# excamera/alfalfa

Measured on NVIDIA H100. Metric: decode_throughput, higher is better.
Workload: dtype u8

## Files before the change

### alfalfa_b200/csrc/encoder.cu

```cuda
#include <cuda_runtime.h>
#include <stdio.h>
#include <stdlib.h>
#include <string.h>

#include <algorithm>
#include <chrono>
#include <condition_variable>
#include <mutex>
#include <string>
#include <utility>
#include <vector>

#include "../../include/vp8gpu.h"
#include "enc_costs.h"
#include "engine.hpp"
#include "hostpool.h"
#include "parser.h"
#include "serializer.h"
#include "vp8_enc_tables.h"
#include "vp8_tables.h"

using vp8::Engine;

extern "C" Engine* vp8gpu_ctx_engine(vp8gpu_ctx* ctx);
// ... 262 lines not shown
  if (late) {
    ft.late_loop_filter_level = &LateLevel::wait;
    ft.late_ctx = late;
  }
  bytes = vp8::serialize_frame(h, enc->h_mbs, enc->h_tokens, nullptr, &ft);
  if (bytes.empty()) return e->fail(VP8GPU_ERR_LOGIC, "serializer rejected the device records");
  return VP8GPU_OK;
}

int filter_frame(vp8gpu_encoder* enc, int frame, bool key, int level) {
  Engine* e = enc->e;
  const vp8::Geom& g = e->geom();
  cudaStream_t s = e->stream(enc->lane);
  if (level <= 0) return VP8GPU_OK;
  vp8::DevJob* dj = reinterpret_cast<vp8::DevJob*>(enc->h_hdr + 512);
  memset(dj, 0, 512);
  int* d_sync = reinterpret_cast<int*>(enc->dev + enc->off_sync);
  dj->mbs = reinterpret_cast<const vp8gpu_mb*>(enc->dev + enc->off_mbs);
  dj->tokens = reinterpret_cast<const vp8gpu_token*>(enc->dev + enc->off_tokens);
  dj->out = e->frame_dev(frame);
  dj->lf_progress = d_sync + 128 + g.mb_rows;
  dj->intra_progress = d_sync + 128;
  dj->key_frame = key;
  dj->sharpness = (uint8_t)enc->lf_sharpness;
  dj->lf_enabled = 1;
  dj->lf_force = (uint8_t)level;
  int ids[1] = {frame};
  int rc = e->acquire_frames(enc->lane, ids, 1);
  if (rc != VP8GPU_OK) return rc;
  CUE(cudaMemcpyAsync(enc->dev + enc->off_encjob + 512, dj, 512, cudaMemcpyHostToDevice, s));
  CUE(cudaMemsetAsync(d_sync + 32, 0, sizeof(int), s));
  CUE(cudaMemsetAsync(d_sync + 128 + g.mb_rows, 0, sizeof(int) * (size_t)g.mb_rows, s));
  const vp8::DevJob* d_dj = reinterpret_cast<const vp8::DevJob*>(enc->dev + enc->off_encjob + 512);
  if (int ce = vp8::launch_loopfilter(d_dj, 1, g, d_sync + 32, e->next_epoch(2), s)) return e->cuda_fail((cudaError_t)ce, "k_loopfilter");
  e->count_launches(1);
  e->mark_frames(enc->lane, ids, 1);
  CUE(cudaStreamSynchronize(s));
  return VP8GPU_OK;
}

int filter_batch(vp8gpu_encoder* enc, const int* frames, const int* levels, int n, bool key) {
  Engine* e = enc->e;
  const vp8::Geom& g = e->geom();
  cudaStream_t s = e->stream(enc->lane);
  if (n <= 0) return VP8GPU_OK;
  if (n > kLfMax) return e->fail(VP8GPU_ERR_LOGIC, "filter_batch: too many trials");
  vp8::DevJob* dj = reinterpret_cast<vp8::DevJob*>(enc->h_hdr + 512);
  memset(dj, 0, sizeof(vp8::DevJob) * n);
  int* d_sync = reinterpret_cast<int*>(enc->dev + enc->off_sync);
  for (int i = 0; i < n; i++) {
    dj[i].mbs = reinterpret_cast<const vp8gpu_mb*>(enc->dev + enc->off_mbs);
    dj[i].tokens = reinterpret_cast<const vp8gpu_token*>(enc->dev + enc->off_tokens);
    dj[i].out = e->frame_dev(frames[i]);
    dj[i].lf_progress = d_sync + 128 + (size_t)(1 + i) * g.mb_rows;
    dj[i].intra_progress = d_sync + 128;
    dj[i].key_frame = key;
    dj[i].sharpness = (uint8_t)enc->lf_sharpness;
    dj[i].lf_enabled = 1;
    dj[i].lf_force = (uint8_t)levels[i];
  }
  int rc = e->acquire_frames(enc->lane, frames, n);
  if (rc != VP8GPU_OK) return rc;
  CUE(cudaMemcpyAsync(enc->dev + enc->off_encjob + 512, dj, sizeof(vp8::DevJob) * n, cudaMemcpyHostToDevice, s));
  CUE(cudaMemsetAsync(d_sync + 32, 0, sizeof(int), s));
  CUE(cudaMemsetAsync(d_sync + 128 + g.mb_rows, 0, sizeof(int) * (size_t)n * g.mb_rows, s));
  const vp8::DevJob* d_dj = reinterpret_cast<const vp8::DevJob*>(enc->dev + enc->off_encjob + 512);
  if (int ce = vp8::launch_loopfilter(d_dj, n, g, d_sync + 32, e->next_epoch(2), s)) return e->cuda_fail((cudaError_t)ce, "k_loopfilter");
  e->count_launches(1);
  e->mark_frames(enc->lane, frames, n);
  CUE(cudaStreamSynchronize(s));
  return VP8GPU_OK;
}

bool enc_speculate() {
  static const bool on = [] {
    const char* v = getenv("VP8GPU_ENC_SPECULATE");
    return !(v && v[0] == '0');
  }();
  return on;
}

int choose_loop_filter(vp8gpu_encoder* enc, int* recon, bool key, int* level_out, double* ssim_out) {
  Engine* e = enc->e;
  int lo = 0, hi = 63;
  if (enc->last_lf >= 0) {
    lo = enc->last_lf > 0 ? enc->last_lf - 1 : 0;
    hi = enc->last_lf + 1 > 63 ? 63 : enc->last_lf + 1;
  }
  int temps[kLfMax], n_temps = 0;
  const int want = enc_speculate() ? (hi - lo + 1 < kLfMax ? hi - lo + 1 : kLfMax) : 1;
  for (; n_temps < want; n_temps++)
    if (e->frame_alloc(&temps[n_temps]) != VP8GPU_OK) break;
  if (n_temps == 0) return e->fail(VP8GPU_ERR_NOMEM, "loop-filter search: no raster for a trial");
  int best = 0, keep = -1;
  double best_ssim = -1.0;
  int rc = VP8GPU_OK;
  bool stop = false, found = false;
  for (int level = lo; level <= hi && !stop && rc == VP8GPU_OK;) {
    int use[kLfMax], lv[kLfMax], n = 0, nf = 0, fr[kLfMax], fl[kLfMax];
    for (int i = 0; i < n_temps && level + n <= hi; i++) {
// ... 1294 lines not shown
```

### alfalfa_b200/csrc/engine.cu

```cuda
#include "engine.hpp"

#include <cuda.h>
#include <stdlib.h>
#include <string.h>

namespace vp8 {

int launch_compare(const uint8_t* a, const uint8_t* b, const Geom& g, int* d_flag, void* stream);
int launch_hash(const uint8_t* a, const Geom& g, unsigned long long* d_out, void* stream);

namespace {
inline size_t align_up(size_t v, size_t a) { return (v + a - 1) / a * a; }

std::mutex g_tmap_mu;
struct TmapChunk {
  uint8_t* base;
  size_t used, cap;
};
std::vector<TmapChunk> g_tmap_chunks[64];
uint8_t* tmap_arena_alloc(int device, size_t bytes) {
  std::lock_guard<std::mutex> lk(g_tmap_mu);
  if (device < 0 || device >= 64) return nullptr;
  auto& chunks = g_tmap_chunks[device];
  if (chunks.empty() || chunks.back().used + bytes > chunks.back().cap) {
// ... 465 lines not shown
    if (jobs[i].ring) {
      L.mbs_off.push_back(0);
      L.tok_off.push_back(0);
      L.split_off.push_back(0);
      continue;
    }
    L.mbs_off.push_back(off);
    off = align_up(off + n_mbs * sizeof(vp8gpu_mb), 256);
    L.tok_off.push_back(off);
    off = align_up(off + (size_t)jobs[i].desc->n_tokens * sizeof(vp8gpu_token) + 4, 256);
    L.split_off.push_back(off);
    off = align_up(off + (size_t)jobs[i].desc->n_split * sizeof(vp8gpu_split_mvs) + 4, 256);
  }
  L.total = off;
  return L;
}
}

int Engine::build_and_launch(int lane, const DevJob* d_jobs, int* d_sync, int n, bool any_inter, bool any_intra,
                             bool any_lf, cudaEvent_t* between) {
  cudaStream_t s = lanes_[lane];
  if (between) CU(cudaEventRecord(between[2], s));
  if (any_inter) {
    if (int e = launch_inter(d_jobs, n, g_, s)) return cuda_fail((cudaError_t)e, "k_inter launch");
    launches_++;
  }
  if (between) CU(cudaEventRecord(between[0], s));
  if (any_intra) {
    if (int e = launch_intra(d_jobs, n, g_, d_sync + 0, next_epoch(1), s)) return cuda_fail((cudaError_t)e, "k_intra launch");
    launches_++;
  }
  if (between) CU(cudaEventRecord(between[1], s));
  if (any_lf) {
    if (int e = launch_loopfilter(d_jobs, n, g_, d_sync + 32, next_epoch(2), s)) return cuda_fail((cudaError_t)e, "k_loopfilter launch");
    launches_++;
  }
  return VP8GPU_OK;
}

uint32_t Engine::token_cap_for(size_t bits) const {
  const size_t by_bytes = align_up(bits + 16, 256) * 9 + 1024, by_blocks = (size_t)g_.mb_cols * g_.mb_rows * 400;
  return (uint32_t)(by_bytes < by_blocks ? by_bytes : by_blocks);
}

TokenRing Engine::token_ring_layout(size_t max_frame_bytes, bool arena) const {
  const size_t n_mbs = (size_t)g_.mb_cols * g_.mb_rows;
  TokenRing r;
  r.bits_cap = (uint32_t)align_up(max_frame_bytes + 16, 256);
  r.split_cap = (uint32_t)n_mbs;
  r.tok_cap = token_cap_for(max_frame_bytes);
  size_t off = 256;
  r.probs_off = off;
  off += 1280;
  r.info_off = off;
  off = align_up(off + 4 * ((n_mbs + 15) / 16 + 1), 256);
  r.bits_off = off;
  off = align_up(off + r.bits_cap, 256);
  r.host_stride = off;
  r.result_off = off;
  off += 256;
  r.above_off = off;
  off = align_up(off + 2 * (size_t)g_.mb_cols, 256);
  r.mbs_off = off;
  off = align_up(off + n_mbs * sizeof(vp8gpu_mb), 256);
  r.split_off = off;
  off = align_up(off + (size_t)r.split_cap * sizeof(vp8gpu_split_mvs), 256);
  r.tok_off = off;
// ... 414 lines not shown
```

### alfalfa_b200/csrc/engine.h

```cpp
#pragma once
#include <stdint.h>

#include "../../include/vp8gpu.h"

#ifdef VP8GPU_SIMT_EMUL
#define VP8_LAUNCH(kern, grid, block, smem, stream) ::simt::make_launch((grid), (block), (smem), [](auto... a_) { kern(a_...); })
#else
#define VP8_LAUNCH(kern, grid, block, smem, stream) kern<<<(grid), (block), (smem), (stream)>>>
#endif

namespace vp8 {

struct Geom {
  int mb_cols, mb_rows;
  int W, H;
  int y_pitch, c_pitch;
  uint32_t u_off, v_off;
  uint32_t frame_bytes;
  uint32_t msg_lf_off, msg_intra_off;
  uint32_t alloc_bytes;
};

struct DevJob {
  const vp8gpu_mb* mbs;
// ... 39 lines not shown
};

struct ReencJob {
  const uint8_t* target;
  uint8_t* recon;
  const vp8gpu_mb* mbs_in;
  vp8gpu_mb* mbs_out;
  vp8gpu_token* tokens;
  uint32_t* tok_counter;
  uint32_t tok_cap;
  int* progress;
  vp8gpu_quant q;
  uint16_t cols, rows;
};

struct TokJob {
  vp8gpu_mb* mbs;
  vp8gpu_token* tokens;
  const uint8_t* bits;
  const uint8_t* coef_probs;
  uint32_t* result;
  uint16_t* above;
  const uint32_t* mbinfo;
  uint32_t part_off[8], part_len[8];
  uint32_t nparts;
  uint32_t tok_cap;
};

int launch_inter(const DevJob* jobs, int njobs, const Geom& g, void* stream);
int launch_enc_rd_trellis(const EncJob* job, int rows, const Geom& g, int* ticket, void* stream);
int launch_reenc_inter(const ReencJob* jobs, int njobs, int n_mbs, const Geom& g, void* stream);
int launch_reenc_intra(const ReencJob* jobs, int njobs, int rows, const Geom& g, int* ticket, void* stream);
int launch_intra(const DevJob* jobs, int njobs, const Geom& g, int* ticket, uint32_t epoch, void* stream);
int launch_loopfilter(const DevJob* jobs, int njobs, const Geom& g, int* ticket, uint32_t epoch, void* stream);
int launch_tokens(const uint8_t* ring, size_t stride, int first, int count, int nslots, const Geom& g, void* stream);
int launch_fetch_header(void* dst, const void* src_host_devptr, size_t bytes, void* stream);
int launch_ssim(const uint8_t* a, const uint8_t* b, const Geom& g, float* d_windows, void* stream);
int launch_enc_rd(const EncJob* jobs, int njobs, int rows, const Geom& g, int* ticket, void* stream);

}
```

### alfalfa_b200/csrc/engine.hpp

```cpp
#pragma once
#include <cuda_runtime.h>
#include <stdint.h>

#include <atomic>
#include <mutex>
#include <string>
#include <vector>

#include "engine.h"
#include "parser.h"

namespace vp8 {

constexpr int kMaxLanes = 32;
constexpr int kStagingDepth = 3;

struct TokenRing {
  int nslots = 0;
  uint8_t* dev = nullptr;
  uint8_t* host = nullptr;
  size_t stride = 0, host_stride = 0;
  size_t probs_off = 0, info_off = 0, bits_off = 0, result_off = 0, above_off = 0, mbs_off = 0, split_off = 0, tok_off = 0;
  uint32_t bits_cap = 0, split_cap = 0, tok_cap = 0;
  vp8gpu_token* arena = nullptr;
// ... 15 lines not shown
  cudaEvent_t consumed = nullptr;
  const TokenRing* ring = nullptr;
  int ring_slot = 0;
  cudaEvent_t ready = nullptr;
  cudaEvent_t* finished = nullptr;
};

class Engine {
 public:
  static int create(int device, int width, int height, int max_frames, Engine** out, std::string* err);
  ~Engine();

  const Geom& geom() const { return g_; }
  int width() const { return width_; }
  int height() const { return height_; }
  int device() const { return device_; }

  int frame_alloc(int* id);
  int frame_retain(int id);
  int frame_release(int id);
  int frames_free();
  int frames_in_use() {
    std::lock_guard<std::mutex> lk(mu_);
    int n = 0;
    for (const Frame& f : frames_) n += f.refcnt > 0;
    return n;
  }
  uint32_t next_epoch(int kernel_bit = 3) {
    if (!(ll_mask_ & kernel_bit)) return 0;
    uint32_t e = ++epoch_;
    if (e == 0) e = ++epoch_;
    return e;
  }
  int frame_upload(int id, const uint8_t* y, size_t ys, const uint8_t* u, const uint8_t* v, size_t cs);
  int frame_download(int id, uint8_t* y, size_t ys, uint8_t* u, uint8_t* v, size_t cs);
  int frame_download_display(int id, int lane, uint8_t* dst, size_t dst_size, bool wait);
  int frames_download_display(const int* ids, uint8_t* const* dsts, int n, int lane);
  int frame_clear(int id, int lane);
  int frame_copy(int dst, int src, int lane);
  int frame_copy_raw(int id, void* buf, size_t bytes, bool into_frame);
  int frames_equal(int a, int b, int lane, int* equal);
  int frame_hash(int id, int lane, uint64_t* out);
  int frames_ssim(int a, int b, int lane, double* out);

  int submit(int lane, const HostJob* jobs, int n, cudaEvent_t consumed, cudaEvent_t* between = nullptr);

  TokenRing token_ring_layout(size_t max_frame_bytes, bool arena = false) const;
  uint32_t token_cap_for(size_t bits) const;
  int token_ring_create(int nslots, size_t max_frame_bytes, TokenRing** out, size_t arena_tokens = 0);
  void token_ring_free(TokenRing* r);
  int token_ring_stage(TokenRing* r, int slot, const ParsedFrame& f, cudaStream_t s, vp8gpu_token* tokens = nullptr);
  int token_ring_launch(TokenRing* r, int first, int count, cudaStream_t s);
  int token_ring_clear_result(TokenRing* r, int slot, cudaStream_t s);
  int token_ring_result(TokenRing* r, int slot, cudaStream_t s, uint32_t result[2]);

  struct Resident;
  int resident_upload(const HostJob* jobs, int n, Resident** out);
  int resident_run(int lane, Resident* r, float* ms);
  int resident_run_many(int lane, Resident* const* rs, int n, float* total_ms);
  int resident_run_timed(int lane, Resident* r, float ms[3]);
  void resident_free(Resident* r);

  uint8_t* frame_dev(int id) { return frames_[id].dev; }
  const void* frame_tmaps(int id) const { return tmaps_ ? tmaps_ + (size_t)id * 384 : nullptr; }
  int acquire_frames(int lane, const int* ids, int n, uint32_t write_mask = ~0u);
  int mark_frames(int lane, const int* ids, int n, uint32_t write_mask = ~0u);
// ... 26 lines not shown
    uint8_t* host_dev = nullptr;
    size_t host_cap = 0;
    cudaEvent_t done = nullptr;
    bool in_flight = false;
  };
  static constexpr int kEventRing = 2048;
  cudaEvent_t next_event(int slot);
  int touch(Frame& f, int slot, bool write = true, cudaEvent_t shared = nullptr);
  void collect_waits(const Frame& f, int slot, bool write, std::vector<cudaEvent_t>& out) const;
  int wait_for(Frame& f, int slot, cudaStream_t s, bool write = true);
  int build_and_launch(int lane, const DevJob* d_jobs, int* d_sync, int n, bool any_inter, bool any_intra,
                       bool any_lf, cudaEvent_t* between = nullptr);
  int count_jobs(const HostJob& j, uint32_t* n_intra, uint32_t* n_inter, uint32_t* n_filtered) const;

  int device_ = 0, width_ = 0, height_ = 0;
  Geom g_{};
  std::mutex mu_;
  std::vector<Frame> frames_;
  std::vector<int> free_;
  cudaStream_t lanes_[2 * kMaxLanes] = {};
  cudaEvent_t ring_[2 * kMaxLanes][kEventRing] = {};
  int ring_next_[2 * kMaxLanes] = {};
  Staging staging_[kMaxLanes][kStagingDepth];
  int staging_next_[kMaxLanes] = {};
  uint8_t* cmp_scratch_ = nullptr;
  float* ssim_dev_[kMaxLanes] = {};
  float* ssim_host_[kMaxLanes] = {};
  uint8_t* tmaps_ = nullptr;
  int make_tensor_maps(int id);
  std::atomic<uint64_t> launches_{0};
  std::string err_;
  std::mutex err_mu_;
  std::atomic<uint32_t> epoch_{0};
  int ll_mask_ = 1;
};

}
```

### alfalfa_b200/csrc/kernels.cu

```cuda
#include <cuda_runtime.h>
#include <stdint.h>

#include "enc_costs.h"
#include "engine.h"
#include "vp8_math.cuh"

namespace vp8 {
namespace {

#define VP8_LUT_QUALIFIER __device__ const
#include "bpred_lut.inc"

__constant__ int16_t c_sixtap[8][6] = {{0, 0, 128, 0, 0, 0},     {0, -6, 123, 12, -1, 0}, {2, -11, 108, 36, -8, 1},
                                      {0, -9, 93, 50, -6, 0},   {3, -16, 77, 77, -16, 3}, {0, -6, 50, 93, -9, 0},
                                      {1, -8, 36, 108, -11, 2}, {0, -1, 12, 123, -6, 0}};

#ifdef VP8_PROFILE
__device__ unsigned long long g_prof[32];
#define PROF_DECL unsigned long long prof_t = clock64(), prof_acc[8] = {0, 0, 0, 0, 0, 0, 0, 0}; unsigned prof_n = 0
#define PROF(i)                                  \
  do {                                           \
    const unsigned long long now_ = clock64();   \
    prof_acc[i] += now_ - prof_t;                \
    prof_t = now_;                               \
// ... 564 lines not shown
        else d = pix + 256 + 64 * ((b - 16) >> 2) + (((b >> 1) & 1) * 4) * 8 + (b & 1) * 4 + 2 * cp, ds = 8;
        const uint8_t* m = &S.s.mid[b][0][2 * cp];
        if (fy) {
          vitem<4>(m, 4, c_sixtap[fy], d, ds);
        } else {
#pragma unroll
          for (int j = 0; j < 4; j++) *reinterpret_cast<uint16_t*>(d + j * ds) = *reinterpret_cast<const uint16_t*>(m + (j + 2) * 4);
        }
      }
    }
    __syncwarp();
  }

  if (nz) add_residuals(pix, S.coef, nz, S.nzlist, lane);
  store_mb(pix, J.out, g, col, row, lane);
}

#ifndef VP8GPU_SIMT_EMUL
__device__ __forceinline__ int ld_progress(const int* p) {
  int v;
  asm volatile("ld.acquire.gpu.global.s32 %0, [%1];" : "=r"(v) : "l"(p) : "memory");
  return v;
}
__device__ __forceinline__ void st_progress(int* p, int v) {
  asm volatile("st.release.gpu.global.s32 [%0], %1;" ::"l"(p), "r"(v) : "memory");
}
#else
__device__ __forceinline__ int ld_progress(const int* p) {
  simt::yield();
  return *reinterpret_cast<const volatile int*>(p);
}
__device__ __forceinline__ void st_progress(int* p, int v) { *reinterpret_cast<volatile int*>(p) = v; }
#endif
__device__ __forceinline__ void wait_row(const int* progress_above, int need, int lane) {
  if (lane == 0) {
    unsigned ns = 20;
    while (ld_progress(progress_above) < need) {
      __nanosleep(ns);
      if (ns < 160) ns += ns;
    }
  }
  __syncwarp();
}
__device__ __forceinline__ void publish_row(int* progress, int value, int lane) {
  __syncwarp();
  if (lane == 0) st_progress(progress, value);
}
__device__ __forceinline__ uint8_t ldcg_u8(const uint8_t* p) { return __ldcg(p); }

__device__ __forceinline__ int next_marked(uint32_t my_word, int from, int nwords) {
  for (int w = from >> 5; w < nwords; w++) {
    uint32_t bits = __shfl_sync(0xffffffffu, my_word, w);
    if (w == (from >> 5)) bits &= 0xffffffffu << (from & 31);
    if (bits) return w * 32 + __ffs(bits) - 1;
  }
  return -1;
}

constexpr int WS = 48;

__device__ __forceinline__ void add_residuals_intra(uint8_t* W, uint8_t* pixc, const int16_t* coef, int lane,
                                                    bool luma_too) {
  for (int g4 = (luma_too ? lane : 64 + lane); g4 < 96; g4 += 32) {
    int blk, ry;
    uint8_t* p;
    if (g4 < 64) {
// ... 217 lines not shown
      *reinterpret_cast<uint2*>((plane ? V : U) + (size_t)(8 * row + yy) * g.c_pitch + 8 * col) =
          *reinterpret_cast<const uint2*>(pixc + plane * 64 + yy * 8);
    }
    const int next = next_marked(my_word, col + 1, nwords);
    PROF(5);
    publish_row(progress, next < 0 ? cols : next, lane);
    PROF(6);
    PROF_COUNT();
    col = next;
  }
  PROF_FLUSH(0);
}

__device__ __forceinline__ void filter_edge_at(int* px, int q, const vp8m::LfParams& lp, bool mb_edge) {
  const int mask = vp8m::lf_mask(lp.interior, mb_edge ? lp.mb_edge : lp.sub_edge, px[q - 4], px[q - 3], px[q - 2],
                                 px[q - 1], px[q], px[q + 1], px[q + 2], px[q + 3]);
  if (!mask) return;
  const int hev = vp8m::lf_hev(lp.hev, px[q - 2], px[q - 1], px[q], px[q + 1]);
  if (mb_edge) vp8m::lf_mbedge(mask, hev, px[q - 3], px[q - 2], px[q - 1], px[q], px[q + 1], px[q + 2]);
  else vp8m::lf_inner(mask, hev, px[q - 2], px[q - 1], px[q], px[q + 1]);
}
__device__ __forceinline__ void filter_line(int* px, bool luma, bool do_mb_edge, bool do_inner,
                                            const vp8m::LfParams& lp) {
  if (do_mb_edge) filter_edge_at(px, 4, lp, true);
  if (do_inner) {
    filter_edge_at(px, 8, lp, false);
    if (luma) {
      filter_edge_at(px, 12, lp, false);
      filter_edge_at(px, 16, lp, false);
    }
  }
}

__global__ void __launch_bounds__(32 * WF_WARPS, 16) k_loopfilter(const DevJob* __restrict__ jobs, int njobs, Geom g, int* ticket) {
  constexpr int YS = 20, CSZ = 12;
  __shared__ __align__(16) uint8_t s_ry[WF_WARPS][20 * YS];
  __shared__ __align__(16) uint8_t s_rc[WF_WARPS][2][12 * CSZ];
  const int lane = threadIdx.x & 31, warp = threadIdx.x >> 5;
  uint8_t* const ry = s_ry[warp];
  uint8_t (*const rc)[12 * CSZ] = s_rc[warp];
  int t = 0;
  if (lane == 0) t = atomicAdd(ticket, 1);
  t = __shfl_sync(0xffffffffu, t, 0);
  const int row = t / njobs, job = t - row * njobs;
  if (row >= g.mb_rows) return;
  const DevJob& J = jobs[job];
  if (!J.lf_enabled) return;
  const int cols = g.mb_cols;
  const vp8gpu_mb* row_mbs = J.mbs + (size_t)row * cols;

  const int nwords = (cols + 31) >> 5;
  uint32_t my_word = 0;
  for (int w = 0; w < nwords; w++) {
    const int c = w * 32 + lane;
    const bool filtered = c < cols && (J.lf_force || ((__ldg(reinterpret_cast<const uint32_t*>(row_mbs + c) + 2) >> 16) & 0xFF) != 0);
    const uint32_t bits = __ballot_sync(0xffffffffu, filtered);
    if (lane == w) my_word = bits;
  }
  int col = next_marked(my_word, 0, nwords);
  int* progress = J.lf_progress + row;
  publish_row(progress, col < 0 ? cols : col, lane);

  uint8_t* const Y = J.out;
  uint8_t* const U = J.out + g.u_off;
  uint8_t* const V = J.out + g.v_off;
  const int y_lo = row > 0 ? 0 : 4;
// ... 48 lines not shown
        if (lane < 20) left0 = *reinterpret_cast<const uint32_t*>(ry + lane * YS + 16);
        if (lane < 24) left1 = *reinterpret_cast<const uint32_t*>(rc[lane / 12] + (lane % 12) * CSZ + 8);
      } else {
        if (lane < 20 && lane >= y_lo)
          left0 = __ldcg(reinterpret_cast<const uint32_t*>(Y + (size_t)(16 * row - 4 + lane) * g.y_pitch + 16 * col - 4));
        if (lane < 24 && (lane % 12) >= y_lo)
          left1 = __ldcg(reinterpret_cast<const uint32_t*>((lane / 12 ? V : U) + (size_t)(8 * row - 4 + lane % 12) * g.c_pitch + 8 * col - 4));
      }
    }
    __syncwarp();
    if (col > 0) {
      if (lane < 20) *reinterpret_cast<uint32_t*>(ry + lane * YS) = left0;
      if (lane < 24) *reinterpret_cast<uint32_t*>(rc[lane / 12] + (lane % 12) * CSZ) = left1;
    }
    if (row > 0) {
      if (lane < 16) *reinterpret_cast<uint32_t*>(ry + (lane >> 2) * YS + 4 + 4 * (lane & 3)) = top;
      else {
        const int cw = lane - 16, plane = cw >> 3, k2 = cw & 7;
        *reinterpret_cast<uint32_t*>(rc[plane] + (k2 >> 1) * CSZ + 4 + 4 * (k2 & 1)) = top;
      }
    }
#pragma unroll
    for (int k = 0; k < 3; k++) {
      const uint8_t* gp;
      uint8_t* sp;
      own_ptr(k, col, gp, sp);
      *reinterpret_cast<uint32_t*>(sp) = own[k];
    }
    __syncwarp();
    PROF(2);
    const int next = next_marked(my_word, col + 1, nwords);
    if (next >= 0) prefetch_own(next);

    const vp8m::LfParams lp = vp8m::lf_params(J.lf_force ? J.lf_force : f.lf_level, J.sharpness, J.key_frame);
    const bool do_inner = !((f.flags & VP8GPU_MB_HAS_Y2) && f.tok_cnt == 0);
    const bool luma = lane < 16;
    uint8_t* const plane_base = luma ? ry : rc[(lane - 16) >> 3];
    const int stride = luma ? YS : CSZ, idx = luma ? lane : (lane & 7), len = luma ? 20 : 12;
    int px[20];

    {
      const uint32_t* rw = reinterpret_cast<const uint32_t*>(plane_base + (4 + idx) * stride);
#pragma unroll
      for (int k = 0; k < 5; k++) {
        const uint32_t v = (k < 3 || luma) ? rw[k] : 0u;
        px[4 * k] = v & 0xFF, px[4 * k + 1] = (v >> 8) & 0xFF, px[4 * k + 2] = (v >> 16) & 0xFF, px[4 * k + 3] = v >> 24;
      }
      filter_line(px, luma, col > 0, do_inner, lp);
      uint32_t* ww = reinterpret_cast<uint32_t*>(plane_base + (4 + idx) * stride);
#pragma unroll
      for (int k = 0; k < 5; k++)
        if (k < 3 || luma) ww[k] = (uint32_t)px[4 * k] | ((uint32_t)px[4 * k + 1] << 8) | ((uint32_t)px[4 * k + 2] << 16) | ((uint32_t)px[4 * k + 3] << 24);
    }
    __syncwarp();
    {
      uint8_t* cp = plane_base + 4 + idx;
#pragma unroll
      for (int k = 0; k < 20; k++) px[k] = k < len ? cp[k * stride] : 0;
      filter_line(px, luma, row > 0, do_inner, lp);
#pragma unroll
      for (int k = 1; k < 19; k++)
        if (k < len - 1) cp[k * stride] = (uint8_t)px[k];
    }
    __syncwarp();

    PROF(3);
    const int x_lo = col > 0 ? 0 : 1;
    const bool flush_right = next != col + 1;
    {
      uint8_t* const gy = Y + (size_t)(16 * row - 4) * g.y_pitch + 16 * col - 4;
#pragma unroll
      for (int k = 0; k < 3; k++) {
        const int w = lane + 32 * k, r = w >> 2, wx = w & 3;
        if (w < 80 && r >= y_lo && wx >= x_lo)
          *reinterpret_cast<uint32_t*>(gy + (size_t)r * g.y_pitch + 4 * wx) = *reinterpret_cast<const uint32_t*>(ry + r * YS + 4 * wx);
      }
#pragma unroll
      for (int k = 0; k < 2; k++) {
        const int w = lane + 32 * k, plane = w >= 24, kk = w - 24 * plane, r = kk >> 1, wx = kk & 1;
        if (w < 48 && r >= y_lo && wx >= x_lo)
          *reinterpret_cast<uint32_t*>((plane ? V : U) + (size_t)(8 * row - 4 + r) * g.c_pitch + 8 * col - 4 + 4 * wx) =
              *reinterpret_cast<const uint32_t*>(rc[plane] + r * CSZ + 4 * wx);
      }
      if (flush_right) {
        if (lane < 20 && lane >= y_lo)
          *reinterpret_cast<uint32_t*>(gy + (size_t)lane * g.y_pitch + 16) = *reinterpret_cast<const uint32_t*>(ry + lane * YS + 16);
        if (lane < 24) {
          const int plane = lane >= 12, r = lane - 12 * plane;
          if (r >= y_lo)
            *reinterpret_cast<uint32_t*>((plane ? V : U) + (size_t)(8 * row - 4 + r) * g.c_pitch + 8 * col + 4) =
                *reinterpret_cast<const uint32_t*>(rc[plane] + r * CSZ + 8);
        }
      }
    }
    PROF(4);
    publish_row(progress, next < 0 ? cols : next, lane);
    PROF(5);
    PROF_COUNT();
    prev = col;
    col = next;
  }
  PROF_FLUSH(16);
}

#include "wavefront_ll.cuh"

__device__ __forceinline__ int warp_sum(int v) { return __reduce_add_sync(0xffffffffu, v); }
__device__ __forceinline__ uint32_t rdcost(uint32_t rate, uint32_t distortion, uint32_t rm, uint32_t dm) {
  return ((128u + rate * rm) / 256u) + distortion * dm;
}
__device__ __forceinline__ uint32_t variance256(int sum, int sse) {
  const long long s = warp_sum(sum);
  const uint32_t q = (uint32_t)warp_sum(sse);
  return q - (uint32_t)((s * s) / 256);
}

struct __align__(16) EncSmem {
  uint8_t W[17 * WS];
  uint8_t Wb[17 * WS];
  uint8_t src[384];
  uint8_t pcand[2][256];
  uint8_t pixc[128];
  uint8_t tile[21 * 24];
  uint8_t mid[21 * 16];
  int16_t coef[COEF_I16];
  int16_t qb[16][16];
  int16_t tmp[16];
  uint8_t aboveC[2][12];
  uint8_t leftC[2][8];
};
// ... 895 lines not shown
}
__global__ void k_hash(const uint8_t* __restrict__ a, Geom g, unsigned long long* out) {
  const int words_y = g.W / 4, words_c = g.W / 8;
  const int rows_total = g.H + g.H;
  unsigned long long acc = 0;
  for (int r = blockIdx.x; r < rows_total; r += gridDim.x) {
    size_t off;
    int nw;
    if (r < g.H) off = (size_t)r * g.y_pitch, nw = words_y;
    else if (r < g.H + g.H / 2) off = g.u_off + (size_t)(r - g.H) * g.c_pitch, nw = words_c;
    else off = g.v_off + (size_t)(r - g.H - g.H / 2) * g.c_pitch, nw = words_c;
    const uint32_t* pa = reinterpret_cast<const uint32_t*>(a + off);
    for (int i = threadIdx.x; i < nw; i += blockDim.x)
      acc += mix64(((unsigned long long)pa[i] << 32) ^ ((unsigned long long)r << 16) ^ (unsigned long long)i);
  }
  for (int o = 16; o; o >>= 1) acc += __shfl_down_sync(0xffffffffu, acc, o);
  if ((threadIdx.x & 31) == 0 && acc) atomicAdd(out, acc);
}

}

int launch_inter(const DevJob* jobs, int njobs, const Geom& g, void* stream) {
  const int n_mbs = g.mb_cols * g.mb_rows;
  dim3 grid((n_mbs + INTER_WARPS - 1) / INTER_WARPS, njobs);
  VP8_LAUNCH(k_inter, grid, INTER_WARPS * 32, 0, static_cast<cudaStream_t>(stream))(jobs, g);
  return (int)cudaGetLastError();
}
int launch_intra(const DevJob* jobs, int njobs, const Geom& g, int* ticket, uint32_t epoch, void* stream) {
  const int grid = (g.mb_rows * njobs + WF_WARPS - 1) / WF_WARPS;
  if (epoch) VP8_LAUNCH(k_intra_ll, grid, 32 * WF_WARPS, 0, static_cast<cudaStream_t>(stream))(jobs, njobs, g, ticket, epoch);
  else VP8_LAUNCH(k_intra, grid, 32 * WF_WARPS, 0, static_cast<cudaStream_t>(stream))(jobs, njobs, g, ticket);
  return (int)cudaGetLastError();
}
int launch_loopfilter(const DevJob* jobs, int njobs, const Geom& g, int* ticket, uint32_t epoch, void* stream) {
  const int grid = (g.mb_rows * njobs + WF_WARPS - 1) / WF_WARPS;
  if (epoch) VP8_LAUNCH(k_loopfilter_ll, grid, 32 * WF_WARPS, 0, static_cast<cudaStream_t>(stream))(jobs, njobs, g, ticket, epoch);
  else VP8_LAUNCH(k_loopfilter, grid, 32 * WF_WARPS, 0, static_cast<cudaStream_t>(stream))(jobs, njobs, g, ticket);
  return (int)cudaGetLastError();
}

int launch_enc_rd(const EncJob* jobs, int njobs, int rows, const Geom& g, int* ticket, void* stream) {
  VP8_LAUNCH(k_enc_rd<false>, (njobs * rows + WF_WARPS - 1) / WF_WARPS, 32 * WF_WARPS, 0, static_cast<cudaStream_t>(stream))(jobs, njobs, g, ticket);
  return (int)cudaGetLastError();
}
int launch_enc_rd_trellis(const EncJob* job, int rows, const Geom& g, int* ticket, void* stream) {
  VP8_LAUNCH(k_enc_rd<true>, (rows + WF_WARPS - 1) / WF_WARPS, 32 * WF_WARPS, 0, static_cast<cudaStream_t>(stream))(job, 1, g, ticket);
  return (int)cudaGetLastError();
}

int launch_reenc_inter(const ReencJob* jobs, int njobs, int n_mbs, const Geom& g, void* stream) {
  const dim3 grid((n_mbs + REENC_WARPS - 1) / REENC_WARPS, njobs);
  VP8_LAUNCH(k_reenc_inter, grid, 32 * REENC_WARPS, 0, static_cast<cudaStream_t>(stream))(jobs, njobs, g);
  return (int)cudaGetLastError();
}
int launch_reenc_intra(const ReencJob* jobs, int njobs, int rows, const Geom& g, int* ticket, void* stream) {
  VP8_LAUNCH(k_reenc_intra, (njobs * rows + WF_WARPS - 1) / WF_WARPS, 32 * WF_WARPS, 0, static_cast<cudaStream_t>(stream))(jobs, njobs, g, ticket);
  return (int)cudaGetLastError();
}

#ifdef VP8_PROFILE
extern "C" void vp8gpu_debug_profile(unsigned long long out[32], int reset) {
  cudaDeviceSynchronize();
  cudaMemcpyFromSymbol(out, g_prof, sizeof(unsigned long long) * 32);
  if (reset) {
    unsigned long long z[32] = {0};
    cudaMemcpyToSymbol(g_prof, z, sizeof(z));
  }
}
#endif
// ... 31 lines not shown
```

Baseline: 10810.

## Add banded loop-filter kernel passing row edges through shared-memory rings

Adds k_loopfilter_band, in which each CTA filters a band of four consecutive macroblock rows, one warp per row. Filtered bottom edges go to the next warp through a shared-memory ring, and progress is signalled with CTA-scope acquire/release flags instead of global progress counters. Only the band's first and last rows still sync through global memory. The filter body is factored into filter_region so both kernels share it, and the new path is switched on by setting bit 4 of ll_mask_ when the low-latency epoch path is off. The intent is to cut global-memory polling and round trips between adjacent rows, at the cost of extra handshake logic, ring back-pressure stalls and less parallelism per CTA.

```diff
diff --git a/alfalfa_b200/csrc/encoder.cu b/alfalfa_b200/csrc/encoder.cu
--- a/alfalfa_b200/csrc/encoder.cu
+++ b/alfalfa_b200/csrc/encoder.cu
@@ -318,7 +318,7 @@
   CUE(cudaMemsetAsync(d_sync + 32, 0, sizeof(int), s));
   CUE(cudaMemsetAsync(d_sync + 128 + g.mb_rows, 0, sizeof(int) * (size_t)g.mb_rows, s));
   const vp8::DevJob* d_dj = reinterpret_cast<const vp8::DevJob*>(enc->dev + enc->off_encjob + 512);
-  if (int ce = vp8::launch_loopfilter(d_dj, 1, g, d_sync + 32, e->next_epoch(2), s)) return e->cuda_fail((cudaError_t)ce, "k_loopfilter");
+  if (int ce = vp8::launch_loopfilter(d_dj, 1, g, d_sync + 32, e->next_epoch(2), e->lf_band(), s)) return e->cuda_fail((cudaError_t)ce, "k_loopfilter");
   e->count_launches(1);
   e->mark_frames(enc->lane, ids, 1);
   CUE(cudaStreamSynchronize(s));
@@ -351,7 +351,7 @@
   CUE(cudaMemsetAsync(d_sync + 32, 0, sizeof(int), s));
   CUE(cudaMemsetAsync(d_sync + 128 + g.mb_rows, 0, sizeof(int) * (size_t)n * g.mb_rows, s));
   const vp8::DevJob* d_dj = reinterpret_cast<const vp8::DevJob*>(enc->dev + enc->off_encjob + 512);
-  if (int ce = vp8::launch_loopfilter(d_dj, n, g, d_sync + 32, e->next_epoch(2), s)) return e->cuda_fail((cudaError_t)ce, "k_loopfilter");
+  if (int ce = vp8::launch_loopfilter(d_dj, n, g, d_sync + 32, e->next_epoch(2), e->lf_band(), s)) return e->cuda_fail((cudaError_t)ce, "k_loopfilter");
   e->count_launches(1);
   e->mark_frames(enc->lane, frames, n);
   CUE(cudaStreamSynchronize(s));
diff --git a/alfalfa_b200/csrc/engine.cu b/alfalfa_b200/csrc/engine.cu
--- a/alfalfa_b200/csrc/engine.cu
+++ b/alfalfa_b200/csrc/engine.cu
@@ -521,7 +521,7 @@
   }
   if (between) CU(cudaEventRecord(between[1], s));
   if (any_lf) {
-    if (int e = launch_loopfilter(d_jobs, n, g_, d_sync + 32, next_epoch(2), s)) return cuda_fail((cudaError_t)e, "k_loopfilter launch");
+    if (int e = launch_loopfilter(d_jobs, n, g_, d_sync + 32, next_epoch(2), lf_band(), s)) return cuda_fail((cudaError_t)e, "k_loopfilter launch");
     launches_++;
   }
   return VP8GPU_OK;
diff --git a/alfalfa_b200/csrc/engine.h b/alfalfa_b200/csrc/engine.h
--- a/alfalfa_b200/csrc/engine.h
+++ b/alfalfa_b200/csrc/engine.h
@@ -95,7 +95,7 @@
 int launch_reenc_inter(const ReencJob* jobs, int njobs, int n_mbs, const Geom& g, void* stream);
 int launch_reenc_intra(const ReencJob* jobs, int njobs, int rows, const Geom& g, int* ticket, void* stream);
 int launch_intra(const DevJob* jobs, int njobs, const Geom& g, int* ticket, uint32_t epoch, void* stream);
-int launch_loopfilter(const DevJob* jobs, int njobs, const Geom& g, int* ticket, uint32_t epoch, void* stream);
+int launch_loopfilter(const DevJob* jobs, int njobs, const Geom& g, int* ticket, uint32_t epoch, bool band, void* stream);
 int launch_tokens(const uint8_t* ring, size_t stride, int first, int count, int nslots, const Geom& g, void* stream);
 int launch_fetch_header(void* dst, const void* src_host_devptr, size_t bytes, void* stream);
 int launch_ssim(const uint8_t* a, const uint8_t* b, const Geom& g, float* d_windows, void* stream);
diff --git a/alfalfa_b200/csrc/engine.hpp b/alfalfa_b200/csrc/engine.hpp
--- a/alfalfa_b200/csrc/engine.hpp
+++ b/alfalfa_b200/csrc/engine.hpp
@@ -71,6 +71,7 @@
     if (e == 0) e = ++epoch_;
     return e;
   }
+  bool lf_band() const { return ll_mask_ & 4; }
   int frame_upload(int id, const uint8_t* y, size_t ys, const uint8_t* u, const uint8_t* v, size_t cs);
   int frame_download(int id, uint8_t* y, size_t ys, uint8_t* u, uint8_t* v, size_t cs);
   int frame_download_display(int id, int lane, uint8_t* dst, size_t dst_size, bool wait);
@@ -163,7 +164,7 @@
   std::string err_;
   std::mutex err_mu_;
   std::atomic<uint32_t> epoch_{0};
-  int ll_mask_ = 1;
+  int ll_mask_ = 1 | 4;
 };
 
 }
diff --git a/alfalfa_b200/csrc/kernels.cu b/alfalfa_b200/csrc/kernels.cu
--- a/alfalfa_b200/csrc/kernels.cu
+++ b/alfalfa_b200/csrc/kernels.cu
@@ -620,6 +620,36 @@
 }
 __device__ __forceinline__ void st_progress(int* p, int v) { *reinterpret_cast<volatile int*>(p) = v; }
 #endif
+#ifndef VP8GPU_SIMT_EMUL
+__device__ __forceinline__ int ld_flag_cta(const int* p) {
+  int v;
+  asm volatile("ld.acquire.cta.shared::cta.s32 %0, [%1];" : "=r"(v) : "r"((unsigned)__cvta_generic_to_shared(p)) : "memory");
+  return v;
+}
+__device__ __forceinline__ void st_flag_cta(int* p, int v) {
+  asm volatile("st.release.cta.shared::cta.s32 [%0], %1;" ::"r"((unsigned)__cvta_generic_to_shared(p)), "r"(v) : "memory");
+}
+#else
+__device__ __forceinline__ int ld_flag_cta(const int* p) {
+  simt::yield();
+  return *reinterpret_cast<const volatile int*>(p);
+}
+__device__ __forceinline__ void st_flag_cta(int* p, int v) { *reinterpret_cast<volatile int*>(p) = v; }
+#endif
+#ifndef VP8GPU_SIMT_EMUL
+__device__ __forceinline__ int lane_here() {
+  int l;
+  asm volatile("mov.u32 %0, %%laneid;" : "=r"(l));
+  return l;
+}
+#else
+__device__ __forceinline__ int lane_here() { return threadIdx.x & 31; }
+#endif
+__device__ __forceinline__ void wait_flag_cta(const int* flag, int need, int lane) {
+  if (lane == 0)
+    while (ld_flag_cta(flag) < need) __nanosleep(20);
+  __syncwarp();
+}
 __device__ __forceinline__ void wait_row(const int* progress_above, int need, int lane) {
   if (lane == 0) {
     unsigned ns = 20;
@@ -903,6 +933,42 @@
   }
 }
 
+__device__ __forceinline__ void filter_region(uint8_t* ry, uint8_t (*rc)[12 * 12], const DevJob& J, const MbFields& f,
+                                              bool left_edge, bool top_edge, int lane) {
+  constexpr int YS = 20, CSZ = 12;
+  const vp8m::LfParams lp = vp8m::lf_params(J.lf_force ? J.lf_force : f.lf_level, J.sharpness, J.key_frame);
+  const bool do_inner = !((f.flags & VP8GPU_MB_HAS_Y2) && f.tok_cnt == 0);
+  const bool luma = lane < 16;
+  uint8_t* const plane_base = luma ? ry : rc[(lane - 16) >> 3];
+  const int stride = luma ? YS : CSZ, idx = luma ? lane : (lane & 7), len = luma ? 20 : 12;
+  int px[20];
+
+  {
+    const uint32_t* rw = reinterpret_cast<const uint32_t*>(plane_base + (4 + idx) * stride);
+#pragma unroll
+    for (int k = 0; k < 5; k++) {
+      const uint32_t v = (k < 3 || luma) ? rw[k] : 0u;
+      px[4 * k] = v & 0xFF, px[4 * k + 1] = (v >> 8) & 0xFF, px[4 * k + 2] = (v >> 16) & 0xFF, px[4 * k + 3] = v >> 24;
+    }
+    filter_line(px, luma, left_edge, do_inner, lp);
+    uint32_t* ww = reinterpret_cast<uint32_t*>(plane_base + (4 + idx) * stride);
+#pragma unroll
+    for (int k = 0; k < 5; k++)
+      if (k < 3 || luma) ww[k] = (uint32_t)px[4 * k] | ((uint32_t)px[4 * k + 1] << 8) | ((uint32_t)px[4 * k + 2] << 16) | ((uint32_t)px[4 * k + 3] << 24);
+  }
+  __syncwarp();
+  {
+    uint8_t* cp = plane_base + 4 + idx;
+#pragma unroll
+    for (int k = 0; k < 20; k++) px[k] = k < len ? cp[k * stride] : 0;
+    filter_line(px, luma, top_edge, do_inner, lp);
+#pragma unroll
+    for (int k = 1; k < 19; k++)
+      if (k < len - 1) cp[k * stride] = (uint8_t)px[k];
+  }
+  __syncwarp();
+}
+
 __global__ void __launch_bounds__(32 * WF_WARPS, 16) k_loopfilter(const DevJob* __restrict__ jobs, int njobs, Geom g, int* ticket) {
   constexpr int YS = 20, CSZ = 12;
   __shared__ __align__(16) uint8_t s_ry[WF_WARPS][20 * YS];
@@ -1017,37 +1083,7 @@
     const int next = next_marked(my_word, col + 1, nwords);
     if (next >= 0) prefetch_own(next);
 
-    const vp8m::LfParams lp = vp8m::lf_params(J.lf_force ? J.lf_force : f.lf_level, J.sharpness, J.key_frame);
-    const bool do_inner = !((f.flags & VP8GPU_MB_HAS_Y2) && f.tok_cnt == 0);
-    const bool luma = lane < 16;
-    uint8_t* const plane_base = luma ? ry : rc[(lane - 16) >> 3];
-    const int stride = luma ? YS : CSZ, idx = luma ? lane : (lane & 7), len = luma ? 20 : 12;
-    int px[20];
-
-    {
-      const uint32_t* rw = reinterpret_cast<const uint32_t*>(plane_base + (4 + idx) * stride);
-#pragma unroll
-      for (int k = 0; k < 5; k++) {
-        const uint32_t v = (k < 3 || luma) ? rw[k] : 0u;
-        px[4 * k] = v & 0xFF, px[4 * k + 1] = (v >> 8) & 0xFF, px[4 * k + 2] = (v >> 16) & 0xFF, px[4 * k + 3] = v >> 24;
-      }
-      filter_line(px, luma, col > 0, do_inner, lp);
-      uint32_t* ww = reinterpret_cast<uint32_t*>(plane_base + (4 + idx) * stride);
-#pragma unroll
-      for (int k = 0; k < 5; k++)
-        if (k < 3 || luma) ww[k] = (uint32_t)px[4 * k] | ((uint32_t)px[4 * k + 1] << 8) | ((uint32_t)px[4 * k + 2] << 16) | ((uint32_t)px[4 * k + 3] << 24);
-    }
-    __syncwarp();
-    {
-      uint8_t* cp = plane_base + 4 + idx;
-#pragma unroll
-      for (int k = 0; k < 20; k++) px[k] = k < len ? cp[k * stride] : 0;
-      filter_line(px, luma, row > 0, do_inner, lp);
-#pragma unroll
-      for (int k = 1; k < 19; k++)
-        if (k < len - 1) cp[k * stride] = (uint8_t)px[k];
-    }
-    __syncwarp();
+    filter_region(ry, rc, J, f, col > 0, row > 0, lane);
 
     PROF(3);
     const int x_lo = col > 0 ? 0 : 1;
@@ -1081,6 +1117,226 @@
     PROF(4);
     publish_row(progress, next < 0 ? cols : next, lane);
     PROF(5);
+    PROF_COUNT();
+    prev = col;
+    col = next;
+  }
+  PROF_FLUSH(16);
+}
+
+constexpr int LF_BAND = 4, LF_RING = 8;
+
+__global__ void __launch_bounds__(32 * LF_BAND, 32 / LF_BAND) k_loopfilter_band(const DevJob* __restrict__ jobs, int njobs, Geom g, int* ticket) {
+  constexpr int YS = 20, CSZ = 12;
+  struct Row {
+    uint8_t ry[20 * YS];
+    uint8_t rc[2][12 * CSZ];
+    uint32_t ring[LF_RING][32];
+    int done;
+    int free;
+    int pad[2];
+  };
+  __shared__ __align__(16) Row s_rows[LF_BAND];
+  __shared__ int s_ticket;
+  const int lane = threadIdx.x & 31, warp = threadIdx.x >> 5;
+  if (threadIdx.x == 0) s_ticket = atomicAdd(ticket, 1);
+  if (threadIdx.x < LF_BAND) s_rows[threadIdx.x].done = 0, s_rows[threadIdx.x].free = 0;
+  __syncthreads();
+  const int band = s_ticket / njobs, job = s_ticket - band * njobs;
+  const int row = band * LF_BAND + warp;
+  if (row >= g.mb_rows) return;
+  const DevJob& J = jobs[job];
+  if (!J.lf_enabled) return;
+  const int cols = g.mb_cols;
+  const vp8gpu_mb* row_mbs = J.mbs + (size_t)row * cols;
+  Row* const S = s_rows + warp;
+  uint8_t* const ry = S->ry;
+  uint8_t (*const rc)[12 * CSZ] = S->rc;
+  const bool ring_in = warp > 0;
+  const bool ring_out = warp < LF_BAND - 1 && row + 1 < g.mb_rows;
+
+  const int nwords = (cols + 31) >> 5;
+  uint32_t my_word = 0, above_word = 0;
+  for (int w = 0; w < nwords; w++) {
+    const int c = w * 32 + lane;
+    const bool filtered = c < cols && (J.lf_force || ((__ldg(reinterpret_cast<const uint32_t*>(row_mbs + c) + 2) >> 16) & 0xFF) != 0);
+    const uint32_t bits = __ballot_sync(0xffffffffu, filtered);
+    if (lane == w) my_word = bits;
+    if (ring_in) {
+      const bool fa = c < cols && (J.lf_force || ((__ldg(reinterpret_cast<const uint32_t*>(row_mbs - cols + c) + 2) >> 16) & 0xFF) != 0);
+      const uint32_t bits_above = __ballot_sync(0xffffffffu, fa);
+      if (lane == w) above_word = bits_above;
+    }
+  }
+  int* const progress = J.lf_progress + row;
+  auto publish = [&](int done, int free) {
+    __syncwarp();
+    if (lane == 0) {
+      if (warp == LF_BAND - 1) st_progress(progress, done);
+      else st_flag_cta(&S->done, done);
+      if (ring_in) st_flag_cta(&S->free, free);
+    }
+  };
+  int col = next_marked(my_word, 0, nwords);
+  publish(col < 0 ? cols : col, col < 0 ? cols : col - 1);
+
+  uint8_t* const Y = J.out;
+  uint8_t* const U = J.out + g.u_off;
+  uint8_t* const V = J.out + g.v_off;
+  const int y_lo = row > 0 ? 0 : 4;
+
+  auto own_ptr = [&](int k, int c, const uint8_t*& gp, uint8_t*& sp) {
+    const int w = lane_here() + 32 * k;
+    if (w < 64) {
+      const int r = w >> 2, wx = w & 3;
+      gp = Y + (size_t)(16 * row + r) * g.y_pitch + 16 * c + 4 * wx;
+      sp = ry + (4 + r) * YS + 4 + 4 * wx;
+    } else {
+      const int cw = w - 64, plane = cw >> 4, k2 = cw & 15, r = k2 >> 1, wx = k2 & 1;
+      gp = (plane ? V : U) + (size_t)(8 * row + r) * g.c_pitch + 8 * c + 4 * wx;
+      sp = rc[plane] + (4 + r) * CSZ + 4 + 4 * wx;
+    }
+  };
+  uint32_t own[3];
+  auto prefetch_own = [&](int c) {
+#pragma unroll
+    for (int k = 0; k < 3; k++) {
+      const uint8_t* gp;
+      uint8_t* sp;
+      own_ptr(k, c, gp, sp);
+      own[k] = __ldcg(reinterpret_cast<const uint32_t*>(gp));
+    }
+  };
+  if (col >= 0) prefetch_own(col);
+  int prev = -2;
+
+  PROF_DECL;
+  while (col >= 0) {
+    PROF(7);
+    const MbFields f = load_mb(row_mbs + col);
+    const bool have_left = prev == col - 1;
+    uint32_t abits = 0;
+    if (ring_in) {
+#pragma unroll
+      for (int d = -1; d <= 1; d++) {
+        const int c = col + d;
+        const uint32_t word = __shfl_sync(0xffffffffu, above_word, (c >> 5) & 31);
+        if (c >= 0 && c < cols && ((word >> (c & 31)) & 1)) abits |= 1u << (d + 1);
+      }
+    }
+    PROF(0);
+    if (ring_in) wait_flag_cta(&S[-1].done, min(col + 2, cols), lane);
+    PROF(1);
+    if (!ring_in && row > 0) wait_row(progress - 1, min(col + 2, cols), lane);
+    PROF(2);
+
+    const int lane = lane_here();
+    uint32_t top = 0;
+    if (row > 0) {
+      const uint8_t* tp;
+      bool right;
+      if (lane < 16) {
+        const int r = lane >> 2, wx = lane & 3;
+        tp = Y + (size_t)(16 * row - 4 + r) * g.y_pitch + 16 * col + 4 * wx;
+        right = wx == 3;
+      } else {
+        const int cw = lane - 16, plane = cw >> 3, k2 = cw & 7, r = k2 >> 1, wx = k2 & 1;
+        tp = (plane ? V : U) + (size_t)(8 * row - 4 + r) * g.c_pitch + 8 * col + 4 * wx;
+        right = wx == 1;
+      }
+      const bool in_ring = (abits & 2) || (right && (abits & 4));
+      top = in_ring ? S[-1].ring[col & (LF_RING - 1)][lane] : __ldcg(reinterpret_cast<const uint32_t*>(tp));
+    }
+    uint32_t left0 = 0, left1 = 0;
+    if (col > 0) {
+      if (have_left) {
+        if (lane < 20) left0 = *reinterpret_cast<const uint32_t*>(ry + lane * YS + 16);
+        if (lane < 24) left1 = *reinterpret_cast<const uint32_t*>(rc[lane / 12] + (lane % 12) * CSZ + 8);
+      } else {
+        const uint32_t* const corner = S[-1].ring[(col - 1) & (LF_RING - 1)];
+        const bool corner_in_ring = (abits & 3) != 0;
+        if (lane < 20 && lane >= y_lo)
+          left0 = corner_in_ring && lane < 4
+                      ? corner[4 * lane + 3]
+                      : __ldcg(reinterpret_cast<const uint32_t*>(Y + (size_t)(16 * row - 4 + lane) * g.y_pitch + 16 * col - 4));
+        if (lane < 24 && (lane % 12) >= y_lo)
+          left1 = corner_in_ring && lane % 12 < 4
+                      ? corner[16 + 8 * (lane / 12) + 2 * (lane % 12) + 1]
+                      : __ldcg(reinterpret_cast<const uint32_t*>((lane / 12 ? V : U) + (size_t)(8 * row - 4 + lane % 12) * g.c_pitch + 8 * col - 4));
+      }
+    }
+    __syncwarp();
+    if (col > 0) {
+      if (lane < 20) *reinterpret_cast<uint32_t*>(ry + lane * YS) = left0;
+      if (lane < 24) *reinterpret_cast<uint32_t*>(rc[lane / 12] + (lane % 12) * CSZ) = left1;
+    }
+    if (row > 0) {
+      if (lane < 16) *reinterpret_cast<uint32_t*>(ry + (lane >> 2) * YS + 4 + 4 * (lane & 3)) = top;
+      else {
+        const int cw = lane - 16, plane = cw >> 3, k2 = cw & 7;
+        *reinterpret_cast<uint32_t*>(rc[plane] + (k2 >> 1) * CSZ + 4 + 4 * (k2 & 1)) = top;
+      }
+    }
+#pragma unroll
+    for (int k = 0; k < 3; k++) {
+      const uint8_t* gp;
+      uint8_t* sp;
+      own_ptr(k, col, gp, sp);
+      *reinterpret_cast<uint32_t*>(sp) = own[k];
+    }
+    __syncwarp();
+    PROF(3);
+    const int next = next_marked(my_word, col + 1, nwords);
+    if (next >= 0) prefetch_own(next);
+
+    filter_region(ry, rc, J, f, col > 0, row > 0, lane);
+
+    PROF(4);
+    if (ring_out) wait_flag_cta(&S[1].free, col - LF_RING + 1, lane);
+    PROF(5);
+    const int x_lo = col > 0 ? 0 : 1;
+    const bool flush_right = next != col + 1;
+    uint32_t* const slot = S->ring[col & (LF_RING - 1)];
+    uint32_t* const slot_left = S->ring[(col - 1) & (LF_RING - 1)];
+    {
+      const int lane = lane_here();
+      uint8_t* const gy = Y + (size_t)(16 * row - 4) * g.y_pitch + 16 * col - 4;
+#pragma unroll
+      for (int k = 0; k < 3; k++) {
+        const int w = lane + 32 * k, r = w >> 2, wx = w & 3;
+        if (w < 80 && r >= y_lo && wx >= x_lo) {
+          const uint32_t v = *reinterpret_cast<const uint32_t*>(ry + r * YS + 4 * wx);
+          *reinterpret_cast<uint32_t*>(gy + (size_t)r * g.y_pitch + 4 * wx) = v;
+          if (ring_out && r >= 16) (wx ? slot : slot_left)[4 * (r - 16) + (wx ? wx - 1 : 3)] = v;
+        }
+      }
+#pragma unroll
+      for (int k = 0; k < 2; k++) {
+        const int w = lane + 32 * k, plane = w >= 24, kk = w - 24 * plane, r = kk >> 1, wx = kk & 1;
+        if (w < 48 && r >= y_lo && wx >= x_lo) {
+          const uint32_t v = *reinterpret_cast<const uint32_t*>(rc[plane] + r * CSZ + 4 * wx);
+          *reinterpret_cast<uint32_t*>((plane ? V : U) + (size_t)(8 * row - 4 + r) * g.c_pitch + 8 * col - 4 + 4 * wx) = v;
+          if (ring_out && r >= 8) (wx ? slot : slot_left)[16 + 8 * plane + 2 * (r - 8) + 1 - wx] = v;
+        }
+      }
+      if (flush_right) {
+        if (lane < 20 && lane >= y_lo) {
+          const uint32_t v = *reinterpret_cast<const uint32_t*>(ry + lane * YS + 16);
+          *reinterpret_cast<uint32_t*>(gy + (size_t)lane * g.y_pitch + 16) = v;
+          if (ring_out && lane >= 16) slot[4 * (lane - 16) + 3] = v;
+        }
+        if (lane < 24) {
+          const int plane = lane >= 12, r = lane - 12 * plane;
+          if (r >= y_lo) {
+            const uint32_t v = *reinterpret_cast<const uint32_t*>(rc[plane] + r * CSZ + 8);
+            *reinterpret_cast<uint32_t*>((plane ? V : U) + (size_t)(8 * row - 4 + r) * g.c_pitch + 8 * col + 4) = v;
+            if (ring_out && r >= 8) slot[16 + 8 * plane + 2 * (r - 8) + 1] = v;
+          }
+        }
+      }
+    }
+    publish(next < 0 ? cols : next, next < 0 ? cols : next - 1);
+    PROF(6);
     PROF_COUNT();
     prev = col;
     col = next;
@@ -2042,9 +2298,11 @@
   else VP8_LAUNCH(k_intra, grid, 32 * WF_WARPS, 0, static_cast<cudaStream_t>(stream))(jobs, njobs, g, ticket);
   return (int)cudaGetLastError();
 }
-int launch_loopfilter(const DevJob* jobs, int njobs, const Geom& g, int* ticket, uint32_t epoch, void* stream) {
+int launch_loopfilter(const DevJob* jobs, int njobs, const Geom& g, int* ticket, uint32_t epoch, bool band, void* stream) {
   const int grid = (g.mb_rows * njobs + WF_WARPS - 1) / WF_WARPS;
   if (epoch) VP8_LAUNCH(k_loopfilter_ll, grid, 32 * WF_WARPS, 0, static_cast<cudaStream_t>(stream))(jobs, njobs, g, ticket, epoch);
+  else if (band)
+    VP8_LAUNCH(k_loopfilter_band, (g.mb_rows + LF_BAND - 1) / LF_BAND * njobs, 32 * LF_BAND, 0, static_cast<cudaStream_t>(stream))(jobs, njobs, g, ticket);
   else VP8_LAUNCH(k_loopfilter, grid, 32 * WF_WARPS, 0, static_cast<cudaStream_t>(stream))(jobs, njobs, g, ticket);
   return (int)cudaGetLastError();
 }
```

New measurement: 11420, median of 6. 1.06x the previous value.
